# zhizdev/sparsefusion

Hardware: AMD Instinct MI355X
Metric: novel views/sec, distillation steps (2 NGP renders fwd+bwd + VAE enc/dec + 51-eval PLMS + LPIPS), 256^2 / 32x32 latents, 2-view synthetic hydrant (higher is better)
Workload: dtype bf16 MFMA operands / f32 accumulate (UNet); f32 (NGP render)

## Files before the change

### sparsefusion_amd/csrc/conv_glds.h

```cpp
#pragma once
#include "conv_lds.h"

template <int BNF, int LDS_BYTES, bool GN, class Pix>
SF_DEV void conv_tile_epilogue(const ConvArgs& a, char* lds, const f32x4 (&acc)[4][BNF / 2], const bool loader, const int wm, const int wn,
                               const int lane, const int nt, const int mt, double* __restrict__ gn_part, const int gn_cg, Pix pix,
                               const int grp = 0) {
  constexpr int WNF = BNF / 2;
  constexpr int COLS = 16 * BNF, F4 = COLS / 4, RPP = 512 / F4, PITCH = COLS + 4;
  static_assert(128 * PITCH * 4 <= LDS_BYTES, "the output tile fits the staging buffers");
  float* ot = reinterpret_cast<float*>(lds);
  sf_lds_barrier();
  if (!loader) {
#pragma unroll
    for (int i = 0; i < 4; ++i)
#pragma unroll
      for (int n = 0; n < WNF; ++n)
#pragma unroll
        for (int r = 0; r < 4; ++r)
          ot[(wm * 64 + i * 16 + (lane >> 4) * 4 + r) * PITCH + (wn * WNF + n) * 16 + (lane & 15)] = acc[i][n][r];
  }
  sf_sync();
  const int tid = threadIdx.x;
  const int c4 = tid % F4, r0 = tid / F4;
  const int col = nt * COLS + c4 * 4;
  const bool cok = col < a.Cout;
  if (a.groups > 1) {
    const long Mrows = (long)a.B * a.Ho * a.Wo;
    if (col < a.npad) {
#pragma unroll 4
      for (int row = r0; row < 128; row += RPP) {
        const long m = pix(row);
        if (m >= 0) *reinterpret_cast<f32x4*>(a.ws + (grp * Mrows + m) * a.npad + col) = *reinterpret_cast<const f32x4*>(ot + row * PITCH + c4 * 4);
      }
    }
    return;
  }
  f32x4 bv = f32x4{0.f, 0.f, 0.f, 0.f};
  if (cok && a.bias) bv = *reinterpret_cast<const f32x4*>(a.bias + col);
  if (a.pixshuf) {
    if (cok) {
      const int hw = a.Ho * a.Wo;
#pragma unroll 4
      for (int row = r0; row < 128; row += RPP) {
        const long m = pix(row);
        if (m < 0) continue;
        const f32x4 v = *reinterpret_cast<const f32x4*>(ot + row * PITCH + c4 * 4) + bv;
        const int b = (int)(m / hw), rr = (int)(m - (long)b * hw);
        const int oy = rr / a.Wo, ox = rr - oy * a.Wo;
        float* o = a.out + (((long)b * (2 * a.Ho) + 2 * oy) * (2 * a.Wo) + 2 * ox) * a.ldc + a.co_off + (col >> 2);
        o[0] = sf_silu(v[0]);
        o[a.ldc] = sf_silu(v[1]);
        o[(long)2 * a.Wo * a.ldc] = sf_silu(v[2]);
        o[(long)(2 * a.Wo + 1) * a.ldc] = sf_silu(v[3]);
      }
    }
    return;
  }
  float gs = 0.0f, gq = 0.0f;
#pragma unroll 4
  for (int row = r0; row < 128; row += RPP) {
    const long m = pix(row);
    if (!cok || m < 0) continue;
    f32x4 v = *reinterpret_cast<const f32x4*>(ot + row * PITCH + c4 * 4) + bv;
    const long o = m * a.ldc + a.co_off + col;
    if (a.resid) v += *reinterpret_cast<const f32x4*>(a.resid + o);
    if (a.accum) v += *reinterpret_cast<const f32x4*>(a.out + o);
    if (a.relu == 1) {
#pragma unroll
      for (int j = 0; j < 4; ++j) v[j] = fmaxf(v[j], 0.0f);
    } else if (a.relu == 2) {
#pragma unroll
      for (int j = 0; j < 4; ++j) v[j] = 0.5f * v[j] * (1.0f + erff(v[j] * 0.70710678118654752f));
    }
    *reinterpret_cast<f32x4*>(a.out + o) = v;
    if (a.ws) {
      bf16x4 tw;
      tw[0] = (sf_opnd)v[0]; tw[1] = (sf_opnd)v[1]; tw[2] = (sf_opnd)v[2]; tw[3] = (sf_opnd)v[3];
      *reinterpret_cast<bf16x4*>(reinterpret_cast<sf_opnd*>(a.ws) + m * a.Cout + col) = tw;
    }
    if (GN) {
#pragma unroll
      for (int j = 0; j < 4; ++j) { gs += v[j]; gq = fmaf(v[j], v[j], gq); }
    }
  }
  if (GN) {
    SF_SHARED float red[2][512];
    red[0][tid] = gs; red[1][tid] = gq;
    sf_sync();
    const int gpt = COLS / gn_cg;
    if (tid < gpt) {
      const int gcol = nt * COLS + tid * gn_cg;
      if (gcol < a.Cout) {
        double s = 0.0, q = 0.0;
        for (int f = tid * (gn_cg >> 2); f < (tid + 1) * (gn_cg >> 2); ++f)
          for (int rr = 0; rr < RPP; ++rr) { s += (double)red[0][rr * F4 + f]; q += (double)red[1][rr * F4 + f]; }
        double* o = gn_part + ((long)mt * (a.Cout / gn_cg) + gcol / gn_cg) * 2;
        o[0] = s; o[1] = q;
      }
    }
  }
}

template <int BNF, int NST, bool GN>
SF_DEV void conv_glds_body(const ConvArgs& a, double* __restrict__ gn_part, const int gn_cg) {
  static_assert(NST == 3 || NST == 4, "ring depth 3 or 4 (the tail of the counted waits is written out for these)");
  static_assert(BNF == 4 || BNF == 8, "64 or 128 output channels per workgroup");
  constexpr int WNF = BNF / 2;
  constexpr int BLD = BNF / 4;
  constexpr int G = 4 + 2 * BLD;
  constexpr int A_BYTES = 8 * 2 * 1024;
  constexpr int STAGE = A_BYTES + BNF * 2 * 1024;
  SF_DYN_LDS(lds);
  const int lane = threadIdx.x & 63, wave = sf_uniform((int)(threadIdx.x >> 6));
  const bool loader = wave >= 4;
  const int wm = (wave >> 1) & 1, wn = wave & 1;
  const int tiles = a.m_tiles * a.n_tiles;
  const int grp = a.groups > 1 ? sf_uniform((int)blockIdx.x / tiles) : 0;
  const int bid = (int)blockIdx.x - grp * tiles;
  int t = bid;
  if (tiles % 8 == 0) t = (bid & 7) * (tiles >> 3) + (bid >> 3);
  const int nt = t % a.n_tiles, mt = t / a.n_tiles;
  const int M = a.B * a.Ho * a.Wo;
  const int S_all = a.KS >> 1;
  const int s_lo = a.groups > 1 ? (int)((long)grp * S_all / a.groups) : 0;
  const int S = (a.groups > 1 ? (int)((long)(grp + 1) * S_all / a.groups) : S_all) - s_lo;

  f32x4 acc[4][WNF];
#pragma unroll
  for (int i = 0; i < 4; ++i)
#pragma unroll
    for (int n = 0; n < WNF; ++n) acc[i][n] = f32x4{0.f, 0.f, 0.f, 0.f};

  if (loader) {
    const int lw = wave - 4;
    int py[4], px[4];
    long pbase[4];
    bool pv[4];
    const int Hs = a.H >> a.ups, Ws = a.W >> a.ups;
#pragma unroll
    for (int q = 0; q < 4; ++q) {
      const int m = (mt * 8 + 2 * lw + (q >> 1)) * 16 + (q & 1) * 8 + (lane >> 3);
      pv[q] = m < M;
      const int mm = pv[q] ? m : 0;
      const int pb = mm / (a.Ho * a.Wo);
      const int r = mm - pb * (a.Ho * a.Wo);
      const int oy = r / a.Wo;
      py[q] = oy * a.stride - a.pad;
      px[q] = (r - oy * a.Wo) * a.stride - a.pad;
      pbase[q] = (long)pb * Hs * Ws;
    }
    int coff[2];
#pragma unroll
    for (int h = 0; h < 2; ++h) coff[h] = ((lane & 7) ^ (((lane >> 4) + 4 * h) & 7)) * 8;
    const sf_opnd* in = reinterpret_cast<const sf_opnd*>(a.in);
    const bf16x8* wbase[BLD];
#pragma unroll
    for (int j = 0; j < BLD; ++j) {
      const int nf = min(nt * BNF + BLD * lw + j, a.n_frags - 1);
      wbase[j] = a.w + (long)nf * a.KS * 64 + lane;
    }
    const int cpairs = a.cchunks >> 1;
    const int tap0 = s_lo / cpairs;
    int i_ks = 2 * s_lo, i_cc = s_lo - tap0 * cpairs, i_ky = tap0 / a.kw, i_kx = tap0 - (tap0 / a.kw) * a.kw, i_buf = 0;
    auto issue_next = [&]() {
      char* sb = lds + i_buf * STAGE;
#pragma unroll
      for (int q = 0; q < 4; ++q) {
        const int iy = py[q] + i_ky, ix = px[q] + i_kx;
        const bool ok = pv[q] & (iy >= 0) & (iy < a.H) & (ix >= 0) & (ix < a.W);
        const int cy = min(max(iy, 0), a.H - 1) >> a.ups, cx = min(max(ix, 0), a.W - 1) >> a.ups;
        const sf_opnd* p = in + ((pbase[q] + (long)cy * Ws + cx) * a.Cin + i_cc * 64 + coff[q & 1]);
        const void* src = ok ? static_cast<const void*>(p) : static_cast<const void*>(sf_zero128 + (lane & 7) * 4);
        sf_glds16(sb + (2 * lw) * 2048 + q * 1024, src);
      }
#pragma unroll
      for (int u = 0; u < 2; ++u)
#pragma unroll
        for (int j = 0; j < BLD; ++j) sf_glds16(sb + A_BYTES + ((BLD * lw + j) * 2 + u) * 1024, wbase[j] + (long)(i_ks + u) * 64);
      i_ks += 2;
      if (++i_cc == cpairs) {
        i_cc = 0;
        if (++i_kx == a.kw) { i_kx = 0; ++i_ky; }
      }
// ... 57 lines not shown
```

### sparsefusion_amd/csrc/conv_halo.h

```cpp
#pragma once
#include "conv_glds.h"

template <int BNF, int NST, bool GN>
SF_DEV void conv_halo_body(const ConvArgs& a, double* __restrict__ gn_part, const int gn_cg) {
  static_assert(NST == 3 || NST == 4, "weight ring depth 3 or 4");
  static_assert(BNF == 4 || BNF == 8, "64 or 128 output channels per workgroup");
  constexpr int WNF = BNF / 2;
  constexpr int G = BNF;
  constexpr int HW_ = 18, HSLOTS = 184;
  constexpr int A_BYTES = HSLOTS * 128, B_STAGE = BNF * 2 * 1024;
  constexpr int LDS_BYTES = 2 * A_BYTES + NST * B_STAGE;
  SF_DYN_LDS(lds);
  const int lane = threadIdx.x & 63, wave = sf_uniform((int)(threadIdx.x >> 6));
  const bool loader = wave >= 4;
  const int wm = (wave >> 1) & 1, wn = wave & 1;
  const int tiles = a.m_tiles * a.n_tiles;
  int t = blockIdx.x;
  if (tiles % 8 == 0) t = (blockIdx.x & 7) * (tiles >> 3) + (blockIdx.x >> 3);
  const int nt = t % a.n_tiles, mt = t / a.n_tiles;
  const int tiles_x = a.W >> 4, tpi = tiles_x * (a.H >> 3);
  const int b = mt / tpi, tr = mt - b * tpi;
  const int ty = tr / tiles_x, y0 = ty * 8, x0 = (tr - ty * tiles_x) * 16;
  const int cpairs = a.cchunks >> 1;
  const int S = 9 * cpairs;

  f32x4 acc[4][WNF];
#pragma unroll
  for (int i = 0; i < 4; ++i)
#pragma unroll
    for (int n = 0; n < WNF; ++n) acc[i][n] = f32x4{0.f, 0.f, 0.f, 0.f};

  if (wave >= 6) {
    const int g0 = (wave - 6) * 12;
    const sf_opnd* src[12];
    int step[12];
#pragma unroll
    for (int j = 0; j < 12; ++j) {
      const int p = (g0 + j) * 8 + (lane >> 3);
      const int hr = p / HW_, hc = p - hr * HW_;
      const int y = y0 - 1 + hr, x = x0 - 1 + hc;
      const bool ok = (p < 10 * HW_) & (y >= 0) & (y < a.H) & (x >= 0) & (x < a.W);
      const int chunk = (lane & 7) ^ (p & 7);
      const int ys = (ok ? y : 0) >> a.ups, xs = (ok ? x : 0) >> a.ups;
      const sf_opnd* in = reinterpret_cast<const sf_opnd*>(a.in) + (((long)b * (a.H >> a.ups) + ys) * (a.W >> a.ups) + xs) * a.Cin + chunk * 8;
      src[j] = ok ? in : reinterpret_cast<const sf_opnd*>(sf_zero128) + (lane & 7) * 8;
      step[j] = ok ? 64 : 0;
    }
    const int nld = wave == 6 ? 12 : 11;
    auto issue_tile = [&](int h) {
      char* ab = lds + (h & 1) * A_BYTES + g0 * 1024;
#pragma unroll
      for (int j = 0; j < 12; ++j)
        if (j < nld) sf_glds16(ab + j * 1024, src[j] + (long)h * step[j]);
    };
    issue_tile(0);
    int tap = 0, h = 0;
    for (int s = 0; s < S; ++s) {
      if (tap == 0) sf_vmcnt<0>();
      sf_lds_barrier();
      if (tap == 0 && h + 1 < cpairs) issue_tile(h + 1);
      if (++tap == 9) { tap = 0; ++h; }
    }
    sf_vmcnt<0>();
    sf_glds_done();
  } else if (wave >= 4) {
    const int lw = wave - 4;
    const bf16x8* wbase[WNF];
#pragma unroll
    for (int j = 0; j < WNF; ++j) {
      const int nf = min(nt * BNF + WNF * lw + j, a.n_frags - 1);
      wbase[j] = a.w + (long)nf * a.KS * 64 + lane;
    }
    int i_tap = 0, i_h = 0, i_buf = 0;
    auto issue_next = [&]() {
      char* sb = lds + 2 * A_BYTES + i_buf * B_STAGE;
      const long kk = (long)i_tap * a.cchunks + 2 * i_h;
#pragma unroll
      for (int u = 0; u < 2; ++u)
#pragma unroll
        for (int j = 0; j < WNF; ++j) sf_glds16(sb + ((WNF * lw + j) * 2 + u) * 1024, wbase[j] + (kk + u) * 64);
      if (++i_tap == 9) { i_tap = 0; ++i_h; }
      if (++i_buf == NST) i_buf = 0;
    };
    for (int p = 0; p < NST - 1 && p < S; ++p) issue_next();
    for (int s = 0; s < S; ++s) {
      const int newer = S - 1 - s;
      if (newer >= NST - 2) sf_vmcnt<G * (NST - 2)>();
      else if (NST == 4 && newer == 1) sf_vmcnt<G>();
      else sf_vmcnt<0>();
      sf_lds_barrier();
      if (s + NST - 1 < S) issue_next();
    }
    sf_vmcnt<0>();
    sf_glds_done();
  } else {
    int aoff[6][3][2];
#pragma unroll
    for (int r = 0; r < 6; ++r)
#pragma unroll
      for (int kx = 0; kx < 3; ++kx) {
        const int p = (wm * 4 + r) * HW_ + kx + (lane & 15);
#pragma unroll
        for (int u = 0; u < 2; ++u) aoff[r][kx][u] = p * 128 + (((u * 4 + (lane >> 4)) ^ (p & 7)) << 4);
      }
    int r_buf = 0;
    SF_LGKM0();
    for (int h = 0; h < cpairs; ++h) {
      const char* ab = lds + (h & 1) * A_BYTES;
#pragma unroll
      for (int tap = 0; tap < 9; ++tap) {
        const int ky = tap / 3, kx = tap - 3 * ky;
        sf_lds_barrier();
        const char* sb = lds + 2 * A_BYTES + r_buf * B_STAGE + lane * 16;
        bf16x8 fa[2][4], fb[2][WNF];
#pragma unroll
        for (int u = 0; u < 2; ++u) {
          fa[u][0] = *reinterpret_cast<const bf16x8*>(ab + aoff[ky][kx][u]);
#pragma unroll
          for (int n = 0; n < WNF; ++n) fb[u][n] = *reinterpret_cast<const bf16x8*>(sb + ((wn * WNF + n) * 2 + u) * 1024);
#pragma unroll
          for (int i = 1; i < 4; ++i) fa[u][i] = *reinterpret_cast<const bf16x8*>(ab + aoff[i + ky][kx][u]);
        }
#pragma unroll
        for (int u = 0; u < 2; ++u)
#pragma unroll
          for (int i = 0; i < 4; ++i)
#pragma unroll
            for (int n = 0; n < WNF; ++n) acc[i][n] = sf_mfma16(fa[u][i], fb[u][n], acc[i][n]);
        constexpr int NRD = 2 * (4 + WNF);
        SF_SCHED_GROUP(0x100, 4);
#pragma unroll
        for (int q = 0; q < NRD - 4; ++q) { SF_SCHED_GROUP(0x008, 1); SF_SCHED_GROUP(0x100, 1); }
        SF_SCHED_GROUP(0x008, 8 * WNF - (NRD - 4));
        if (++r_buf == NST) r_buf = 0;
      }
    }
  }
  conv_tile_epilogue<BNF, LDS_BYTES, GN>(a, lds, acc, loader, wm, wn, lane, nt, mt, gn_part, gn_cg, [&](int row) -> long {
    return ((long)b * a.H + y0 + (row >> 4)) * a.W + x0 + (row & 15);
  });
}

template <int BNF, int NST, bool GN>
SF_KERNEL(512, 1) void k_conv3_halo(ConvArgs a, double* __restrict__ gn_part, int gn_cg) {
  sf_touch_kernarg<(int)sizeof(ConvArgs)>();
  conv_halo_body<BNF, NST, GN>(a, gn_part, gn_cg);
}

static inline uint32_t conv_halo_lds_bytes(int bnf, int nst) { return 2u * 184 * 128 + (uint32_t)nst * bnf * 2 * 1024; }
static inline bool conv_halo_ok(const ConvArgs& a) {
  return a.kh == 3 && a.kw == 3 && a.stride == 1 && a.pad == 1 && a.Ho == a.H && a.Wo == a.W && a.W % 16 == 0 && a.H % 8 == 0 &&
         a.Cin % 64 == 0;
}
```

### sparsefusion_amd/csrc/unet_ops.hip

```cpp

#include "sf_common.h"
#include "plan_ops.h"
#include "sf_dev.h"
#include "gemm_rows.h"
#include "conv_halo.h"
#include "conv_halo_small.h"
#include "conv_igemm.h"
#include "conv_igemm_t.h"
#include "attn_ln.h"
#include <math.h>

typedef __attribute__((ext_vector_type(8))) sf_opnd bf16x8;
typedef __attribute__((ext_vector_type(4))) sf_opnd bf16x4;
typedef __attribute__((ext_vector_type(4))) float f32x4;
typedef __attribute__((address_space(1))) float gfloat;

__device__ __forceinline__ void atomic_add_f32(float* p, float v) {
  (void)__builtin_amdgcn_global_atomic_fadd_f32((gfloat*)p, v);
}
__device__ __forceinline__ float silu_f(float v) { return v / (1.0f + __expf(-v)); }
__device__ __forceinline__ float sigmoid_f(float v) { return 1.0f / (1.0f + __expf(-v)); }
__device__ __forceinline__ float gelu_f(float v) { return 0.5f * v * (1.0f + erff(v * 0.70710678118654752f)); }

__device__ __forceinline__ float wave_sum(float v) {
// ... 375 lines not shown
  const int lane = threadIdx.x & 63, wv = threadIdx.x >> 6;
  float mx = -INFINITY;
  for (int i = threadIdx.x; i < N; i += 256) mx = fmaxf(mx, x[i] * scale);
  mx = wave_max(mx);
  if (lane == 0) red[wv] = mx;
  __syncthreads();
  mx = fmaxf(fmaxf(red[0], red[1]), fmaxf(red[2], red[3]));
  float s = 0.0f;
  for (int i = threadIdx.x; i < N; i += 256) s += expf(x[i] * scale - mx);
  s = wave_sum(s);
  if (lane == 0) red[4 + wv] = s;
  __syncthreads();
  const float inv = 1.0f / (red[4] + red[5] + red[6] + red[7]);
  for (int i = threadIdx.x; i < N; i += 256) out[(long)blockIdx.x * N + i] = (sf_opnd)(expf(x[i] * scale - mx) * inv);
}

__global__ __launch_bounds__(256) void k_unpack_out(const float* __restrict__ in, float* __restrict__ out, int B, int HW,
                                                    int C, int ldi) {
  const long n = (long)B * C * HW;
  for (long i = blockIdx.x * 256L + threadIdx.x; i < n; i += (long)gridDim.x * 256) {
    const int p = (int)(i % HW);
    const long bc = i / HW;
    const int c = (int)(bc % C), b = (int)(bc / C);
    out[i] = in[((long)b * HW + p) * ldi + c];
  }
}
__global__ __launch_bounds__(256) void k_add(const float* __restrict__ a, float* __restrict__ out, long n) {
  for (long i = blockIdx.x * 256L + threadIdx.x; i < n; i += (long)gridDim.x * 256) out[i] += a[i];
}

__global__ void k_time_emb(const float* __restrict__ t, const float* __restrict__ w, float* __restrict__ out, int B,
                           int half) {
  const int i = blockIdx.x * blockDim.x + threadIdx.x;
  if (i >= B * half) return;
  const int b = i / half, j = i - b * half;
  const float fr = t[b] * w[j] * 2.0f * 3.14159265358979323846f;
  float* o = out + (long)b * (1 + 2 * half);
  if (j == 0) o[0] = t[b];
  o[1 + j] = sinf(fr);
  o[1 + half + j] = cosf(fr);
}

template <int WM, int WN>
static void launch_conv(const ConvArgs& a, bool a_fp32, int blocks, hipStream_t st) {
  if (a_fp32) k_conv_igemm<WM, WN, true><<<blocks, 256, 0, st>>>(a);
  else k_conv_igemm<WM, WN, false><<<blocks, 256, 0, st>>>(a);
}

static unsigned long long g_igemm_t_launches = 0;
extern "C" uint64_t sf_conv_igemm_t_launches(void) { return g_igemm_t_launches; }
static bool launch_conv_t(const ConvArgs& a, int WM, int WN, bool a_fp32, int blocks, hipStream_t st) {
  if (a.B != 1 || a.H != a.W || a.kh != a.kw || a.accum || a.resid || a.relu || a.co_off) return false;
  const int epi = a.pixshuf ? SF_IGT_PIXSHUF : SF_IGT_SPLITK;
  if (a.pixshuf ? (!a.slots_out || !a.bias || a.ldc * 4 != a.Cout || a.groups != 1) : (a.groups < 2 || !a.ws)) return false;
#define SF_TRY_IGT(hl_, cin_, cout_, k_, s_, p_, ups_, wm_, wn_, g_, f32_, epi_) \
  if (a.H == (1 << hl_) && a.Cin == cin_ && a.Cout == cout_ && a.kh == k_ && a.stride == s_ && a.pad == p_ && a.ups == ups_ && WM == wm_ && \
      WN == wn_ && a.groups == g_ && a_fp32 == (bool)f32_ && epi == epi_ && a.Ho == ((1 << hl_) + 2 * p_ - k_) / s_ + 1 && a.Wo == a.Ho) { \
    k_conv_igemm_t<hl_, cin_, cout_, k_, s_, p_, ups_, wm_, wn_, g_, (bool)f32_, epi_><<<blocks, 256, 0, st>>>(a); \
    ++g_igemm_t_launches; \
    return true; \
  }
  SF_IGEMM_T_VARIANTS(SF_TRY_IGT)
#undef SF_TRY_IGT
  return false;
}

static int conv_glds_depth() { return 4; }
template <int BNF, int NST, bool GN>
static int launch_conv_glds(const ConvArgs& a, int nblk, double* part, int cg, hipStream_t st) {
  static unsigned mask = 0;
  const uint32_t lds = conv_glds_lds_bytes(BNF, NST);
  int dev = 0;
  if (hipGetDevice(&dev) != hipSuccess) SF_FAIL(SF_ERR_LAUNCH, "hipGetDevice failed");
  if (dev >= 32 || !(mask & (1u << dev))) {
    if (hipFuncSetAttribute(reinterpret_cast<const void*>(&k_conv_glds<BNF, NST, GN>), hipFuncAttributeMaxDynamicSharedMemorySize, (int)lds) != hipSuccess)
      SF_FAIL(SF_ERR_LAUNCH, "hipFuncSetAttribute(max dynamic LDS) failed");
    if (dev < 32) mask |= 1u << dev;
  }
  k_conv_glds<BNF, NST, GN><<<nblk, 512, lds, st>>>(a, part, cg);
  SF_CHECK_LAUNCH("conv_glds");
  return SF_OK;
}
static bool conv_halo_enabled() { return true; }
template <int BNF, int NST, bool GN>
static int launch_conv_halo(const ConvArgs& a, int nblk, double* part, int cg, hipStream_t st) {
  static unsigned mask = 0;
  const uint32_t lds = conv_halo_lds_bytes(BNF, NST);
  int dev = 0;
  if (hipGetDevice(&dev) != hipSuccess) SF_FAIL(SF_ERR_LAUNCH, "hipGetDevice failed");
  if (dev >= 32 || !(mask & (1u << dev))) {
    if (hipFuncSetAttribute(reinterpret_cast<const void*>(&k_conv3_halo<BNF, NST, GN>), hipFuncAttributeMaxDynamicSharedMemorySize, (int)lds) != hipSuccess)
      SF_FAIL(SF_ERR_LAUNCH, "hipFuncSetAttribute(max dynamic LDS) failed");
    if (dev < 32) mask |= 1u << dev;
  }
  k_conv3_halo<BNF, NST, GN><<<nblk, 512, lds, st>>>(a, part, cg);
  SF_CHECK_LAUNCH("conv3_halo");
  return SF_OK;
}
template <int BNF, bool GN>
static int launch_conv_halo_nst(const ConvArgs& a, int nblk, double* part, int cg, int nst, hipStream_t st) {
  return nst == 3 ? launch_conv_halo<BNF, 3, GN>(a, nblk, part, cg, st) : launch_conv_halo<BNF, 4, GN>(a, nblk, part, cg, st);
}

template <int BNF, int NST, int MAPL>
static int launch_conv_halo_sm(const ConvArgs& a, int nblk, hipStream_t st) {
  static unsigned mask = 0;
  const uint32_t lds = conv_halo_sm_lds_bytes(BNF, NST, MAPL);
  int dev = 0;
  if (hipGetDevice(&dev) != hipSuccess) SF_FAIL(SF_ERR_LAUNCH, "hipGetDevice failed");
  if (dev >= 32 || !(mask & (1u << dev))) {
    if (hipFuncSetAttribute(reinterpret_cast<const void*>(&k_conv3_halo_sm<BNF, NST, MAPL>), hipFuncAttributeMaxDynamicSharedMemorySize, (int)lds) != hipSuccess)
      SF_FAIL(SF_ERR_LAUNCH, "hipFuncSetAttribute(max dynamic LDS) failed");
    if (dev < 32) mask |= 1u << dev;
  }
  k_conv3_halo_sm<BNF, NST, MAPL><<<nblk, 512, lds, st>>>(a);
  SF_CHECK_LAUNCH("conv3_halo_sm");
  return SF_OK;
}
template <int BNF>
static int launch_conv_halo_sm_nst(const ConvArgs& a, int nblk, int nst, hipStream_t st) {
  if (a.H == 4) return nst == 3 ? launch_conv_halo_sm<BNF, 3, 2>(a, nblk, st) : launch_conv_halo_sm<BNF, 4, 2>(a, nblk, st);
  return nst == 3 ? launch_conv_halo_sm<BNF, 3, 3>(a, nblk, st) : launch_conv_halo_sm<BNF, 4, 3>(a, nblk, st);
}

template <int BNF, bool GN>
static int launch_conv_glds_nst(const ConvArgs& a, int nblk, double* part, int cg, int nst, hipStream_t st) {
  return nst == 3 ? launch_conv_glds<BNF, 3, GN>(a, nblk, part, cg, st) : launch_conv_glds<BNF, 4, GN>(a, nblk, part, cg, st);
}

static int conv_splitk_tail(const sf_op& op, const ConvArgs& a, int M, hipStream_t st) {
  if (a.groups <= 1) return SF_OK;
  if (!a.ws) SF_FAIL(SF_ERR_INVALID, "conv: split-K needs a workspace");
  if (op.flags & 8) return SF_OK;
  k_splitk_reduce<<<sf_grid_cap(sf_div_up((long)M * a.Cout, 256)), 256, 0, st>>>(a.ws, a.bias, a.resid, a.out, M, a.Cout, a.npad,
                                                                                a.groups, a.ldc, a.co_off, a.accum, a.relu, a.out_nchw_hw);
  SF_CHECK_LAUNCH("splitk_reduce");
  return SF_OK;
}

static int run_conv(const sf_op& op, hipStream_t st) {
  ConvArgs a;
  a.in = op.p[0]; a.w = (const bf16x8*)op.p[1]; a.bias = (const float*)op.p[2]; a.out = (float*)op.p[3];
  a.resid = (const float*)op.p[4]; a.ws = (float*)op.p[5];
  a.accum = (op.flags & 4) ? 1 : 0;
  a.B = op.i[0]; a.H = op.i[1]; a.W = op.i[2]; a.Cin = op.i[3]; a.Ho = op.i[4]; a.Wo = op.i[5]; a.Cout = op.i[6];
  a.ldc = op.i[7]; a.co_off = op.i[8]; a.kh = op.i[9]; a.kw = op.i[10]; a.stride = op.i[11]; a.pad = op.i[12];
  a.groups = op.i[13] > 0 ? op.i[13] : 1;
  const int tile = op.i[14];
  const int WM = tile / 16, WN = tile % 16;
  a.pixshuf = (op.flags & 2) ? 1 : 0;
  a.slots_out = (float*)op.p[7];
  a.out_nchw_hw = (op.flags & 256) ? op.i[4] * op.i[5] : 0;
  a.ups = (op.flags & 16) ? 1 : 0;
  a.relu = (op.flags & 32) ? 1 : ((op.flags & 64) ? 2 : 0);
  if (a.ups && ((a.H | a.W) & 1)) SF_FAIL(SF_ERR_INVALID, "conv: upsampled input dims must be even");
  if (a.Cin % 32) SF_FAIL(SF_ERR_INVALID, "conv: Cin_pad must be a multiple of 32");
  if (a.pixshuf && a.groups != 1) SF_FAIL(SF_ERR_INVALID, "conv: pixel-shuffle epilogue cannot be split-K");
  a.cchunks = a.Cin / 32;
  a.KS = a.kh * a.kw * a.cchunks;
  const int M = a.B * a.Ho * a.Wo;
  a.m_frags = (M + 15) / 16;
  a.n_frags = (a.Cout + 15) / 16;
  a.m_tiles = (a.m_frags + WM - 1) / WM;
  a.n_tiles = (a.n_frags + WN - 1) / WN;
  a.npad = a.n_frags * 16;
  if (a.pixshuf) a.groups = 1;
  if (a.slots_out && (!a.pixshuf || tile >= 256 || (a.Cout / 4) % 16 || a.ldc % 16 || a.co_off % 16 || M % 16 || (a.Ho * a.Wo) % 16))
    SF_FAIL(SF_ERR_INVALID, "conv: output slots ride on the pixel-shuffle epilogue only (16 | Cout / 4, ldc, co_off, Ho * Wo)");
  if (a.out_nchw_hw && (a.groups < 2 || (op.flags & (8 | 4)) || op.p[4] || tile >= 256 || a.co_off || a.ldc != a.Cout))
    SF_FAIL(SF_ERR_INVALID, "conv: NCHW output is written by the (non-deferred) split-K reduction of a plain conv only");
  a.steps_per_wave = (a.KS + a.groups * 4 - 1) / (a.groups * 4);
  const int blocks = a.m_tiles * a.n_tiles * a.groups;
  const bool f32 = (op.flags & 1) != 0;
  if (tile >= 256) {
    const int bnf = (tile - 256) & 15, sel = (tile - 256) >> 4;
    if (sel != 0 && sel != 1 && sel != 3 && sel != 4 && sel != 6 && sel != 7 && sel != 8 && sel != 9)
      SF_FAIL(SF_ERR_INVALID, "conv: unknown LDS kernel selector %d", sel);
    const bool glds_ok = !f32 && a.Cin % 64 == 0 && a.Cout % 4 == 0 && a.ldc % 4 == 0 && a.co_off % 4 == 0 && (bnf == 8 || bnf == 4);
    if (sel >= 3 && !glds_ok) SF_FAIL(SF_ERR_INVALID, "conv: k_conv_glds takes operand-type activations with Cin %% 64 == 0 and float4-aligned output rows only");
    const bool special = a.groups != 1 || a.pixshuf;
    if (special && ((op.flags & 128) || sel == 6 || sel == 7 || (a.groups != 1 && !a.ws) || (a.pixshuf && ((op.flags & 4) || op.p[4] || a.relu))))
      SF_FAIL(SF_ERR_INVALID, "conv: split-K / pixel shuffle on the LDS-tiled kernels: no GroupNorm partials, not k_conv3_halo; no residual / accumulate / ReLU under the shuffle");
    const bool sm_ok = glds_ok && conv_halo_sm_ok(a) && !a.pixshuf && !(op.flags & 128);
    if (sel >= 8 && !sm_ok) SF_FAIL(SF_ERR_INVALID, "conv: k_conv3_halo_sm takes 3x3 / stride 1 / pad 1 layers on 4x4 / 8x8 maps, groups <= Cin / 64");
    const int sm = sel >= 8 ? sel - 5 : ((sel == 0 && sm_ok) ? conv_glds_depth() : 0);
    if (!sm && a.groups > (((glds_ok && sel != 1) ? a.KS : a.KS + 1) >> 1)) SF_FAIL(SF_ERR_INVALID, "conv: more split-K groups than stages");
    if (a.groups == 1 && a.pixshuf) a.ws = nullptr;
    a.m_tiles = (a.m_frags + 7) / 8;
    a.n_tiles = (a.n_frags + bnf - 1) / bnf;
    const int nblk = a.m_tiles * a.n_tiles * a.groups;
    const bool halo_ok = glds_ok && conv_halo_ok(a) && M % 128 == 0 && !special;
    if ((sel == 6 || sel == 7) && !halo_ok) SF_FAIL(SF_ERR_INVALID, "conv: k_conv3_halo takes 3x3 / stride 1 / pad 1 layers with W %% 16 == 0, H %% 8 == 0 only");
    if (sm) {
      if (int rc = bnf == 8 ? launch_conv_halo_sm_nst<8>(a, nblk, sm, st) : launch_conv_halo_sm_nst<4>(a, nblk, sm, st)) return rc;
      return conv_splitk_tail(op, a, M, st);
    }
    const int glds = (glds_ok && sel != 1 && sel < 6) ? (sel >= 3 ? sel : conv_glds_depth()) : 0;
    const int halo = (sel == 6 || sel == 7) ? sel - 3 : ((sel == 0 && halo_ok && glds && conv_halo_enabled()) ? glds : 0);
    if (op.flags & 128) {
      double* part = (double*)op.p[6];
      const int cg = op.i[15];
      if (!part || (cg != 4 && cg != 8 && cg != 16) || a.Cout % cg || a.co_off || a.ldc != a.Cout || (a.Ho * a.Wo) % 128)
        SF_FAIL(SF_ERR_INVALID, "conv: GroupNorm-partials epilogue needs whole rows, 128 | Ho*Wo, group width 4 / 8 / 16");
      if (halo) return bnf == 8 ? launch_conv_halo_nst<8, true>(a, nblk, part, cg, halo, st) : launch_conv_halo_nst<4, true>(a, nblk, part, cg, halo, st);
      if (glds) return bnf == 8 ? launch_conv_glds_nst<8, true>(a, nblk, part, cg, glds, st) : launch_conv_glds_nst<4, true>(a, nblk, part, cg, glds, st);
      if (bnf == 8) {
        if (f32) k_conv_lds_gn<8, true><<<nblk, 256, 0, st>>>(a, part, cg); else k_conv_lds_gn<8, false><<<nblk, 256, 0, st>>>(a, part, cg);
      } else if (bnf == 4) {
        if (f32) k_conv_lds_gn<4, true><<<nblk, 256, 0, st>>>(a, part, cg); else k_conv_lds_gn<4, false><<<nblk, 256, 0, st>>>(a, part, cg);
      } else {
        SF_FAIL(SF_ERR_INVALID, "conv: unsupported LDS tile %d", bnf);
      }
      SF_CHECK_LAUNCH("conv_lds_gn");
      return SF_OK;
    }
    if (halo) return bnf == 8 ? launch_conv_halo_nst<8, false>(a, nblk, nullptr, 0, halo, st) : launch_conv_halo_nst<4, false>(a, nblk, nullptr, 0, halo, st);
    if (glds) {
      if (int rc = bnf == 8 ? launch_conv_glds_nst<8, false>(a, nblk, nullptr, 0, glds, st) : launch_conv_glds_nst<4, false>(a, nblk, nullptr, 0, glds, st)) return rc;
      return conv_splitk_tail(op, a, M, st);
    }
    if (bnf == 8) {
      if (f32) k_conv_lds<8, true><<<nblk, 256, 0, st>>>(a); else k_conv_lds<8, false><<<nblk, 256, 0, st>>>(a);
    } else if (bnf == 4) {
      if (f32) k_conv_lds<4, true><<<nblk, 256, 0, st>>>(a); else k_conv_lds<4, false><<<nblk, 256, 0, st>>>(a);
    } else {
      SF_FAIL(SF_ERR_INVALID, "conv: unsupported LDS tile %d", bnf);
    }
    SF_CHECK_LAUNCH("conv_lds");
    return conv_splitk_tail(op, a, M, st);
  }
  if ((op.flags & 512) && launch_conv_t(a, WM, WN, f32, blocks, st)) {
    SF_CHECK_LAUNCH("conv_igemm_t");
    return conv_splitk_tail(op, a, M, st);
  }
  switch (tile) {
    case 1 * 16 + 1: launch_conv<1, 1>(a, f32, blocks, st); break;
    case 1 * 16 + 2: launch_conv<1, 2>(a, f32, blocks, st); break;
    case 1 * 16 + 4: launch_conv<1, 4>(a, f32, blocks, st); break;
    case 2 * 16 + 1: launch_conv<2, 1>(a, f32, blocks, st); break;
    case 2 * 16 + 2: launch_conv<2, 2>(a, f32, blocks, st); break;
    case 2 * 16 + 4: launch_conv<2, 4>(a, f32, blocks, st); break;
    case 4 * 16 + 1: launch_conv<4, 1>(a, f32, blocks, st); break;
    case 4 * 16 + 2: launch_conv<4, 2>(a, f32, blocks, st); break;
    case 4 * 16 + 4: launch_conv<4, 4>(a, f32, blocks, st); break;
    default: SF_FAIL(SF_ERR_INVALID, "conv: unsupported wave tile %dx%d", WM, WN);
  }
  SF_CHECK_LAUNCH("conv_igemm");
  return conv_splitk_tail(op, a, M, st);
}

static int lazy_from_op(const sf_op& op, int ibase, int M, LazySrc& lz) {
  lz.mode = op.i[ibase]; lz.groups = op.i[ibase + 1]; lz.npad = op.i[ibase + 2]; lz.M = M;
  lz.a = (const float*)op.p[8]; lz.b = (const float*)op.p[9]; lz.r = (const float*)op.p[10];
  if (lz.mode < 0 || lz.mode > 2) SF_FAIL(SF_ERR_INVALID, "lazy source: unknown mode %d", lz.mode);
  if (lz.mode && !lz.a) SF_FAIL(SF_ERR_INVALID, "lazy source: missing operand");
  if (lz.mode == 1 && (lz.groups < 1 || lz.npad % 4)) SF_FAIL(SF_ERR_INVALID, "lazy source: bad split-K geometry");
  if (lz.mode == 2 && !lz.b) SF_FAIL(SF_ERR_INVALID, "lazy source: gate missing");
  return SF_OK;
}

static int run_gn(const sf_op& op, hipStream_t st) {
  const int B = op.i[0], HW = op.i[1], C1 = op.i[2], C2 = op.i[3];
  const int C = C1 + C2, G = op.i[8] > 0 ? op.i[8] : 8;
  if (C % (4 * G) || C1 % 4 || !op.p[7])
    SF_FAIL(SF_ERR_INVALID, "gn_act: unsupported shape HW=%d C=%d G=%d (or missing stats buffer)", HW, C, G);
  const int chunks = HW * (C / G) / 4;
  LazySrc lz;
  if (int rc = lazy_from_op(op, 5, B * HW, lz)) return rc;
  const int c4 = C / 4;
  if (!(op.flags & (2 | 4)) && (B * G >= 256 || (B * G >= 64 && (long)B * HW * C <= (1L << 19)) || (op.flags & 8)) && chunks <= 1024 * 16) {
    float* s1 = (float*)op.p[0];
    const float *s2 = (const float*)op.p[1], *ga = (const float*)op.p[2], *be = (const float*)op.p[3], *ssp = (const float*)op.p[4];
    sf_opnd *o = (sf_opnd*)op.p[5], *rw = (sf_opnd*)op.p[6];
#define SF_GN_ONE(NT, NCH) k_gn_one<NT, NCH><<<B * G, NT, 0, st>>>(s1, s2, ga, be, ssp, o, rw, HW, C1, C2, op.i[4], op.f[0], op.f[1], op.flags & 1, lz, G)
    if (chunks <= 256 * 2) SF_GN_ONE(256, 2);
    else if (chunks <= 256 * 4) SF_GN_ONE(256, 4);
    else if (chunks <= 256 * 8) SF_GN_ONE(256, 8);
    else if (chunks <= 256 * 16) SF_GN_ONE(256, 16);
    else if (chunks <= 1024 * 8) SF_GN_ONE(1024, 8);
    else SF_GN_ONE(1024, 16);
#undef SF_GN_ONE
    SF_CHECK_LAUNCH("gn_one");
    return SF_OK;
  }
  if (op.flags & 2) {
    if (op.p[1] || lz.mode) SF_FAIL(SF_ERR_INVALID, "gn_act: ready-made statistics need a plain single source");
  } else if (!op.p[1] && !lz.mode && C / G <= 16 && c4 <= 256 && 256 % c4 == 0) {
    const int ppi = 256 / c4;
    int slabs = HW / (ppi * 16);
    slabs = slabs < 1 ? 1 : (slabs > 1024 ? 1024 : slabs);
    k_gn_stats_px<<<B * slabs, 256, 0, st>>>((const float*)op.p[0], (double*)op.p[7], HW, C, G, slabs);
  } else {
    const int per_block = lz.mode == 1 ? 256 : GN_CHUNKS_PER_BLOCK;
    int slices = (chunks + per_block - 1) / per_block;
    const int want = 128 / (B * G), max_slices = (chunks + 255) / 256;
    if (slices < want) slices = want < max_slices ? want : max_slices;
    if (slices < 1) slices = 1;
    k_gn_stats<<<B * G * slices, 256, 0, st>>>((float*)op.p[0], (const float*)op.p[1], (double*)op.p[7], HW, C1, C2, slices,
                                               op.f[1], lz, G);
// ... 374 lines not shown
```

Measured before the change: 18.14.

## Shrink halo conv pixel tile height when the grid underfills the GPU

Templates the halo 3x3 conv kernel on the pixel-tile height (8, 4 or 2 rows) and picks a smaller height automatically when the 8-row grid has fewer than 192 workgroups, so small feature maps put more workgroups on the device's compute units. Because the GroupNorm-partial epilogue assumes 128-row tiles, the small-tile path writes output first and then runs a separate kernel that rereads the output to compute the GN partials. The trade-off is lower weight reuse per workgroup, an extra global read and an extra launch on the GN path.

```diff
diff --git a/sparsefusion_amd/csrc/conv_glds.h b/sparsefusion_amd/csrc/conv_glds.h
--- a/sparsefusion_amd/csrc/conv_glds.h
+++ b/sparsefusion_amd/csrc/conv_glds.h
@@ -1,23 +1,45 @@
 #pragma once
 #include "conv_lds.h"
 
-template <int BNF, int LDS_BYTES, bool GN, class Pix>
-SF_DEV void conv_tile_epilogue(const ConvArgs& a, char* lds, const f32x4 (&acc)[4][BNF / 2], const bool loader, const int wm, const int wn,
+template <int BNF>
+SF_DEV void conv_tile_gn_reduce(const float gs, const float gq, const int tid, const int nt, const int mt, const int Cout,
+                                double* __restrict__ gn_part, const int gn_cg) {
+  constexpr int COLS = 16 * BNF, F4 = COLS / 4, RPP = 512 / F4;
+  SF_SHARED float red[2][512];
+  red[0][tid] = gs; red[1][tid] = gq;
+  sf_sync();
+  const int gpt = COLS / gn_cg;
+  if (tid < gpt) {
+    const int gcol = nt * COLS + tid * gn_cg;
+    if (gcol < Cout) {
+      double s = 0.0, q = 0.0;
+      for (int f = tid * (gn_cg >> 2); f < (tid + 1) * (gn_cg >> 2); ++f)
+        for (int rr = 0; rr < RPP; ++rr) { s += (double)red[0][rr * F4 + f]; q += (double)red[1][rr * F4 + f]; }
+      double* o = gn_part + ((long)mt * (Cout / gn_cg) + gcol / gn_cg) * 2;
+      o[0] = s; o[1] = q;
+    }
+  }
+}
+
+template <int BNF, int LDS_BYTES, bool GN, class Pix, int MI>
+SF_DEV void conv_tile_epilogue(const ConvArgs& a, char* lds, const f32x4 (&acc)[MI][BNF / 2], const bool loader, const int wm, const int wn,
                                const int lane, const int nt, const int mt, double* __restrict__ gn_part, const int gn_cg, Pix pix,
                                const int grp = 0) {
   constexpr int WNF = BNF / 2;
   constexpr int COLS = 16 * BNF, F4 = COLS / 4, RPP = 512 / F4, PITCH = COLS + 4;
-  static_assert(128 * PITCH * 4 <= LDS_BYTES, "the output tile fits the staging buffers");
+  constexpr int ROWS = 32 * MI;
+  static_assert(MI == 4 || (!GN && (MI == 2 || MI == 1)), "128-row tiles; 64 / 32 rows without GroupNorm partial sums");
+  static_assert(ROWS * PITCH * 4 <= LDS_BYTES, "the output tile fits the staging buffers");
   float* ot = reinterpret_cast<float*>(lds);
   sf_lds_barrier();
   if (!loader) {
 #pragma unroll
-    for (int i = 0; i < 4; ++i)
+    for (int i = 0; i < MI; ++i)
 #pragma unroll
       for (int n = 0; n < WNF; ++n)
 #pragma unroll
         for (int r = 0; r < 4; ++r)
-          ot[(wm * 64 + i * 16 + (lane >> 4) * 4 + r) * PITCH + (wn * WNF + n) * 16 + (lane & 15)] = acc[i][n][r];
+          ot[(wm * (16 * MI) + i * 16 + (lane >> 4) * 4 + r) * PITCH + (wn * WNF + n) * 16 + (lane & 15)] = acc[i][n][r];
   }
   sf_sync();
   const int tid = threadIdx.x;
@@ -28,7 +50,7 @@
     const long Mrows = (long)a.B * a.Ho * a.Wo;
     if (col < a.npad) {
 #pragma unroll 4
-      for (int row = r0; row < 128; row += RPP) {
+      for (int row = r0; row < ROWS; row += RPP) {
         const long m = pix(row);
         if (m >= 0) *reinterpret_cast<f32x4*>(a.ws + (grp * Mrows + m) * a.npad + col) = *reinterpret_cast<const f32x4*>(ot + row * PITCH + c4 * 4);
       }
@@ -41,7 +63,7 @@
     if (cok) {
       const int hw = a.Ho * a.Wo;
 #pragma unroll 4
-      for (int row = r0; row < 128; row += RPP) {
+      for (int row = r0; row < ROWS; row += RPP) {
         const long m = pix(row);
         if (m < 0) continue;
         const f32x4 v = *reinterpret_cast<const f32x4*>(ot + row * PITCH + c4 * 4) + bv;
@@ -58,7 +80,7 @@
   }
   float gs = 0.0f, gq = 0.0f;
 #pragma unroll 4
-  for (int row = r0; row < 128; row += RPP) {
+  for (int row = r0; row < ROWS; row += RPP) {
     const long m = pix(row);
     if (!cok || m < 0) continue;
     f32x4 v = *reinterpret_cast<const f32x4*>(ot + row * PITCH + c4 * 4) + bv;
@@ -83,22 +105,30 @@
       for (int j = 0; j < 4; ++j) { gs += v[j]; gq = fmaf(v[j], v[j], gq); }
     }
   }
-  if (GN) {
-    SF_SHARED float red[2][512];
-    red[0][tid] = gs; red[1][tid] = gq;
-    sf_sync();
-    const int gpt = COLS / gn_cg;
-    if (tid < gpt) {
-      const int gcol = nt * COLS + tid * gn_cg;
-      if (gcol < a.Cout) {
-        double s = 0.0, q = 0.0;
-        for (int f = tid * (gn_cg >> 2); f < (tid + 1) * (gn_cg >> 2); ++f)
-          for (int rr = 0; rr < RPP; ++rr) { s += (double)red[0][rr * F4 + f]; q += (double)red[1][rr * F4 + f]; }
-        double* o = gn_part + ((long)mt * (a.Cout / gn_cg) + gcol / gn_cg) * 2;
-        o[0] = s; o[1] = q;
-      }
-    }
-  }
+  if (GN) conv_tile_gn_reduce<BNF>(gs, gq, tid, nt, mt, a.Cout, gn_part, gn_cg);
+}
+
+template <int BNF>
+SF_KERNEL(512) void k_conv_gn_partials(const float* __restrict__ out, double* __restrict__ gn_part, int H, int W, int Cout, int n_tiles, int gn_cg) {
+  constexpr int COLS = 16 * BNF, F4 = COLS / 4, RPP = 512 / F4;
+  const int tid = threadIdx.x;
+  const int nt = blockIdx.x % n_tiles, mt = blockIdx.x / n_tiles;
+  const int tiles_x = W >> 4, tpi = tiles_x * (H >> 3);
+  const int b = mt / tpi, tr = mt - b * tpi;
+  const int ty = tr / tiles_x, y0 = ty * 8, x0 = (tr - ty * tiles_x) * 16;
+  const int c4 = tid % F4, r0 = tid / F4;
+  const int col = nt * COLS + c4 * 4;
+  float gs = 0.0f, gq = 0.0f;
+  if (col < Cout) {
+#pragma unroll 4
+    for (int row = r0; row < 128; row += RPP) {
+      const long m = ((long)b * H + y0 + (row >> 4)) * W + x0 + (row & 15);
+      const f32x4 v = *reinterpret_cast<const f32x4*>(out + m * Cout + col);
+#pragma unroll
+      for (int j = 0; j < 4; ++j) { gs += v[j]; gq = fmaf(v[j], v[j], gq); }
+    }
+  }
+  conv_tile_gn_reduce<BNF>(gs, gq, tid, nt, mt, Cout, gn_part, gn_cg);
 }
 
 template <int BNF, int NST, bool GN>
diff --git a/sparsefusion_amd/csrc/conv_halo.h b/sparsefusion_amd/csrc/conv_halo.h
--- a/sparsefusion_amd/csrc/conv_halo.h
+++ b/sparsefusion_amd/csrc/conv_halo.h
@@ -1,13 +1,16 @@
 #pragma once
 #include "conv_glds.h"
 
-template <int BNF, int NST, bool GN>
+template <int BNF, int NST, bool GN, int TH = 8>
 SF_DEV void conv_halo_body(const ConvArgs& a, double* __restrict__ gn_part, const int gn_cg) {
   static_assert(NST == 3 || NST == 4, "weight ring depth 3 or 4");
   static_assert(BNF == 4 || BNF == 8, "64 or 128 output channels per workgroup");
+  static_assert(TH == 8 || ((TH == 4 || TH == 2) && !GN), "pixel tile of 8 rows, or 4 / 2 without GroupNorm partial sums");
   constexpr int WNF = BNF / 2;
+  constexpr int MI = TH / 2;
   constexpr int G = BNF;
-  constexpr int HW_ = 18, HSLOTS = 184;
+  constexpr int HW_ = 18, HROWS = TH + 2;
+  constexpr int NLD = (HROWS * HW_ + 7) / 8, NLW = (NLD + 1) / 2, HSLOTS = NLD * 8;
   constexpr int A_BYTES = HSLOTS * 128, B_STAGE = BNF * 2 * 1024;
   constexpr int LDS_BYTES = 2 * A_BYTES + NST * B_STAGE;
   SF_DYN_LDS(lds);
@@ -18,39 +21,39 @@
   int t = blockIdx.x;
   if (tiles % 8 == 0) t = (blockIdx.x & 7) * (tiles >> 3) + (blockIdx.x >> 3);
   const int nt = t % a.n_tiles, mt = t / a.n_tiles;
-  const int tiles_x = a.W >> 4, tpi = tiles_x * (a.H >> 3);
+  const int tiles_x = a.W >> 4, tpi = tiles_x * (a.H / TH);
   const int b = mt / tpi, tr = mt - b * tpi;
-  const int ty = tr / tiles_x, y0 = ty * 8, x0 = (tr - ty * tiles_x) * 16;
+  const int ty = tr / tiles_x, y0 = ty * TH, x0 = (tr - ty * tiles_x) * 16;
   const int cpairs = a.cchunks >> 1;
   const int S = 9 * cpairs;
 
-  f32x4 acc[4][WNF];
+  f32x4 acc[MI][WNF];
 #pragma unroll
-  for (int i = 0; i < 4; ++i)
+  for (int i = 0; i < MI; ++i)
 #pragma unroll
     for (int n = 0; n < WNF; ++n) acc[i][n] = f32x4{0.f, 0.f, 0.f, 0.f};
 
   if (wave >= 6) {
-    const int g0 = (wave - 6) * 12;
-    const sf_opnd* src[12];
-    int step[12];
+    const int g0 = (wave - 6) * NLW;
+    const sf_opnd* src[NLW];
+    int step[NLW];
 #pragma unroll
-    for (int j = 0; j < 12; ++j) {
+    for (int j = 0; j < NLW; ++j) {
       const int p = (g0 + j) * 8 + (lane >> 3);
       const int hr = p / HW_, hc = p - hr * HW_;
       const int y = y0 - 1 + hr, x = x0 - 1 + hc;
-      const bool ok = (p < 10 * HW_) & (y >= 0) & (y < a.H) & (x >= 0) & (x < a.W);
+      const bool ok = (p < HROWS * HW_) & (y >= 0) & (y < a.H) & (x >= 0) & (x < a.W);
       const int chunk = (lane & 7) ^ (p & 7);
       const int ys = (ok ? y : 0) >> a.ups, xs = (ok ? x : 0) >> a.ups;
       const sf_opnd* in = reinterpret_cast<const sf_opnd*>(a.in) + (((long)b * (a.H >> a.ups) + ys) * (a.W >> a.ups) + xs) * a.Cin + chunk * 8;
       src[j] = ok ? in : reinterpret_cast<const sf_opnd*>(sf_zero128) + (lane & 7) * 8;
       step[j] = ok ? 64 : 0;
     }
-    const int nld = wave == 6 ? 12 : 11;
+    const int nld = wave == 6 ? NLW : NLD - NLW;
     auto issue_tile = [&](int h) {
       char* ab = lds + (h & 1) * A_BYTES + g0 * 1024;
 #pragma unroll
-      for (int j = 0; j < 12; ++j)
+      for (int j = 0; j < NLW; ++j)
         if (j < nld) sf_glds16(ab + j * 1024, src[j] + (long)h * step[j]);
     };
     issue_tile(0);
@@ -94,12 +97,12 @@
     sf_vmcnt<0>();
     sf_glds_done();
   } else {
-    int aoff[6][3][2];
+    int aoff[MI + 2][3][2];
 #pragma unroll
-    for (int r = 0; r < 6; ++r)
+    for (int r = 0; r < MI + 2; ++r)
 #pragma unroll
       for (int kx = 0; kx < 3; ++kx) {
-        const int p = (wm * 4 + r) * HW_ + kx + (lane & 15);
+        const int p = (wm * MI + r) * HW_ + kx + (lane & 15);
 #pragma unroll
         for (int u = 0; u < 2; ++u) aoff[r][kx][u] = p * 128 + (((u * 4 + (lane >> 4)) ^ (p & 7)) << 4);
       }
@@ -112,26 +115,26 @@
         const int ky = tap / 3, kx = tap - 3 * ky;
         sf_lds_barrier();
         const char* sb = lds + 2 * A_BYTES + r_buf * B_STAGE + lane * 16;
-        bf16x8 fa[2][4], fb[2][WNF];
+        bf16x8 fa[2][MI], fb[2][WNF];
 #pragma unroll
         for (int u = 0; u < 2; ++u) {
           fa[u][0] = *reinterpret_cast<const bf16x8*>(ab + aoff[ky][kx][u]);
 #pragma unroll
           for (int n = 0; n < WNF; ++n) fb[u][n] = *reinterpret_cast<const bf16x8*>(sb + ((wn * WNF + n) * 2 + u) * 1024);
 #pragma unroll
-          for (int i = 1; i < 4; ++i) fa[u][i] = *reinterpret_cast<const bf16x8*>(ab + aoff[i + ky][kx][u]);
+          for (int i = 1; i < MI; ++i) fa[u][i] = *reinterpret_cast<const bf16x8*>(ab + aoff[i + ky][kx][u]);
         }
 #pragma unroll
         for (int u = 0; u < 2; ++u)
 #pragma unroll
-          for (int i = 0; i < 4; ++i)
+          for (int i = 0; i < MI; ++i)
 #pragma unroll
             for (int n = 0; n < WNF; ++n) acc[i][n] = sf_mfma16(fa[u][i], fb[u][n], acc[i][n]);
-        constexpr int NRD = 2 * (4 + WNF);
+        constexpr int NRD = 2 * (MI + WNF);
         SF_SCHED_GROUP(0x100, 4);
 #pragma unroll
         for (int q = 0; q < NRD - 4; ++q) { SF_SCHED_GROUP(0x008, 1); SF_SCHED_GROUP(0x100, 1); }
-        SF_SCHED_GROUP(0x008, 8 * WNF - (NRD - 4));
+        SF_SCHED_GROUP(0x008, 2 * MI * WNF - (NRD - 4));
         if (++r_buf == NST) r_buf = 0;
       }
     }
@@ -141,13 +144,15 @@
   });
 }
 
-template <int BNF, int NST, bool GN>
+template <int BNF, int NST, bool GN, int TH = 8>
 SF_KERNEL(512, 1) void k_conv3_halo(ConvArgs a, double* __restrict__ gn_part, int gn_cg) {
   sf_touch_kernarg<(int)sizeof(ConvArgs)>();
-  conv_halo_body<BNF, NST, GN>(a, gn_part, gn_cg);
+  conv_halo_body<BNF, NST, GN, TH>(a, gn_part, gn_cg);
 }
 
-static inline uint32_t conv_halo_lds_bytes(int bnf, int nst) { return 2u * 184 * 128 + (uint32_t)nst * bnf * 2 * 1024; }
+static inline uint32_t conv_halo_lds_bytes(int bnf, int nst, int th = 8) {
+  return 2u * (((th + 2) * 18 + 7) / 8) * 1024 + (uint32_t)nst * bnf * 2 * 1024;
+}
 static inline bool conv_halo_ok(const ConvArgs& a) {
   return a.kh == 3 && a.kw == 3 && a.stride == 1 && a.pad == 1 && a.Ho == a.H && a.Wo == a.W && a.W % 16 == 0 && a.H % 8 == 0 &&
          a.Cin % 64 == 0;
diff --git a/sparsefusion_amd/csrc/unet_ops.hip b/sparsefusion_amd/csrc/unet_ops.hip
--- a/sparsefusion_amd/csrc/unet_ops.hip
+++ b/sparsefusion_amd/csrc/unet_ops.hip
@@ -481,18 +481,18 @@
   return SF_OK;
 }
 static bool conv_halo_enabled() { return true; }
-template <int BNF, int NST, bool GN>
+template <int BNF, int NST, bool GN, int TH = 8>
 static int launch_conv_halo(const ConvArgs& a, int nblk, double* part, int cg, hipStream_t st) {
   static unsigned mask = 0;
-  const uint32_t lds = conv_halo_lds_bytes(BNF, NST);
+  const uint32_t lds = conv_halo_lds_bytes(BNF, NST, TH);
   int dev = 0;
   if (hipGetDevice(&dev) != hipSuccess) SF_FAIL(SF_ERR_LAUNCH, "hipGetDevice failed");
   if (dev >= 32 || !(mask & (1u << dev))) {
-    if (hipFuncSetAttribute(reinterpret_cast<const void*>(&k_conv3_halo<BNF, NST, GN>), hipFuncAttributeMaxDynamicSharedMemorySize, (int)lds) != hipSuccess)
+    if (hipFuncSetAttribute(reinterpret_cast<const void*>(&k_conv3_halo<BNF, NST, GN, TH>), hipFuncAttributeMaxDynamicSharedMemorySize, (int)lds) != hipSuccess)
       SF_FAIL(SF_ERR_LAUNCH, "hipFuncSetAttribute(max dynamic LDS) failed");
     if (dev < 32) mask |= 1u << dev;
   }
-  k_conv3_halo<BNF, NST, GN><<<nblk, 512, lds, st>>>(a, part, cg);
+  k_conv3_halo<BNF, NST, GN, TH><<<nblk, 512, lds, st>>>(a, part, cg);
   SF_CHECK_LAUNCH("conv3_halo");
   return SF_OK;
 }
@@ -500,6 +500,14 @@
 static int launch_conv_halo_nst(const ConvArgs& a, int nblk, double* part, int cg, int nst, hipStream_t st) {
   return nst == 3 ? launch_conv_halo<BNF, 3, GN>(a, nblk, part, cg, st) : launch_conv_halo<BNF, 4, GN>(a, nblk, part, cg, st);
 }
+template <int BNF>
+static int launch_conv_halo_th(ConvArgs a, int nst, int th, hipStream_t st) {
+  a.m_tiles = a.m_frags / th;
+  const int nblk = a.m_tiles * a.n_tiles;
+  if (th == 4) return nst == 3 ? launch_conv_halo<BNF, 3, false, 4>(a, nblk, nullptr, 0, st) : launch_conv_halo<BNF, 4, false, 4>(a, nblk, nullptr, 0, st);
+  return nst == 3 ? launch_conv_halo<BNF, 3, false, 2>(a, nblk, nullptr, 0, st) : launch_conv_halo<BNF, 4, false, 2>(a, nblk, nullptr, 0, st);
+}
+static int conv_halo_tile_rows(int blocks8) { return blocks8 >= 192 ? 8 : (2 * blocks8 >= 192 ? 4 : 2); }
 
 template <int BNF, int NST, int MAPL>
 static int launch_conv_halo_sm(const ConvArgs& a, int nblk, hipStream_t st) {
@@ -572,7 +580,10 @@
   const int blocks = a.m_tiles * a.n_tiles * a.groups;
   const bool f32 = (op.flags & 1) != 0;
   if (tile >= 256) {
-    const int bnf = (tile - 256) & 15, sel = (tile - 256) >> 4;
+    const int bnf = (tile - 256) & 15, sel = ((tile - 256) >> 4) & 255;
+    const int thc = (tile - 256) >> 12;
+    if (thc && (thc > 2 || (sel != 6 && sel != 7)))
+      SF_FAIL(SF_ERR_INVALID, "conv: a pixel-tile height goes with k_conv3_halo (selectors 6 / 7) only");
     if (sel != 0 && sel != 1 && sel != 3 && sel != 4 && sel != 6 && sel != 7 && sel != 8 && sel != 9)
       SF_FAIL(SF_ERR_INVALID, "conv: unknown LDS kernel selector %d", sel);
     const bool glds_ok = !f32 && a.Cin % 64 == 0 && a.Cout % 4 == 0 && a.ldc % 4 == 0 && a.co_off % 4 == 0 && (bnf == 8 || bnf == 4);
@@ -601,6 +612,14 @@
       const int cg = op.i[15];
       if (!part || (cg != 4 && cg != 8 && cg != 16) || a.Cout % cg || a.co_off || a.ldc != a.Cout || (a.Ho * a.Wo) % 128)
         SF_FAIL(SF_ERR_INVALID, "conv: GroupNorm-partials epilogue needs whole rows, 128 | Ho*Wo, group width 4 / 8 / 16");
+      const int th = !halo ? 8 : (sel ? 8 >> thc : conv_halo_tile_rows(nblk));
+      if (th < 8) {
+        if (int rc = bnf == 8 ? launch_conv_halo_th<8>(a, halo, th, st) : launch_conv_halo_th<4>(a, halo, th, st)) return rc;
+        if (bnf == 8) k_conv_gn_partials<8><<<nblk, 512, 0, st>>>(a.out, part, a.H, a.W, a.Cout, a.n_tiles, cg);
+        else k_conv_gn_partials<4><<<nblk, 512, 0, st>>>(a.out, part, a.H, a.W, a.Cout, a.n_tiles, cg);
+        SF_CHECK_LAUNCH("conv_gn_partials");
+        return SF_OK;
+      }
       if (halo) return bnf == 8 ? launch_conv_halo_nst<8, true>(a, nblk, part, cg, halo, st) : launch_conv_halo_nst<4, true>(a, nblk, part, cg, halo, st);
       if (glds) return bnf == 8 ? launch_conv_glds_nst<8, true>(a, nblk, part, cg, glds, st) : launch_conv_glds_nst<4, true>(a, nblk, part, cg, glds, st);
       if (bnf == 8) {
@@ -613,7 +632,11 @@
       SF_CHECK_LAUNCH("conv_lds_gn");
       return SF_OK;
     }
-    if (halo) return bnf == 8 ? launch_conv_halo_nst<8, false>(a, nblk, nullptr, 0, halo, st) : launch_conv_halo_nst<4, false>(a, nblk, nullptr, 0, halo, st);
+    if (halo) {
+      const int th = sel ? 8 >> thc : conv_halo_tile_rows(nblk);
+      if (th < 8) return bnf == 8 ? launch_conv_halo_th<8>(a, halo, th, st) : launch_conv_halo_th<4>(a, halo, th, st);
+      return bnf == 8 ? launch_conv_halo_nst<8, false>(a, nblk, nullptr, 0, halo, st) : launch_conv_halo_nst<4, false>(a, nblk, nullptr, 0, halo, st);
+    }
     if (glds) {
       if (int rc = bnf == 8 ? launch_conv_glds_nst<8, false>(a, nblk, nullptr, 0, glds, st) : launch_conv_glds_nst<4, false>(a, nblk, nullptr, 0, glds, st)) return rc;
       return conv_splitk_tail(op, a, M, st);
```

Result: no change. 17.97 (-0.9%).
